# limanling/clip-event

Measured on AMD Instinct MI355X. Metric: image-text pairs/sec/GPU, ViT-B/32 224px x 77-tok, global-batch contrastive, higher is better.
Workload: dtype bf16; 1 GPU; ViT-B/32 224px x 77-tok, bf16 operands, per-GPU batch 256, K=1, InfoNCE only, full train step (fwd+bwd+clip_grad_norm+Adam), random-init weights; global_batch=256, parallelism=dp1, captions=SOT + U[8,75] random ids + EOT, zero-padded to 77 (SURVEY 8(d) c2), text_rows=live tokens SOT..EOT only: 54.8% of B*77 rows (identical results, see DESIGN.md), fresh_captions_every_step=True, alignment=False, cu_hog=0, nt_pgrid=256, full=False

## Files before the change

### clip_event_amd/csrc/attention.hip

```cpp
#include <map>
#include <mutex>

#include <type_traits>

#include "common.hpp"
#include "../../include/clip_event_hip.h"

namespace {

constexpr int HD = 64;
constexpr int ROW = 160;

typedef __attribute__((address_space(3))) s16x4 lds_s16x4;
typedef __attribute__((ext_vector_type(8))) short s16x8;

__device__ __forceinline__ bf16x8 tr_pair(const char* p0, const char* p1) {
    s16x4 lo = __builtin_amdgcn_ds_read_tr16_b64_v4i16((lds_s16x4*)p0);
    s16x4 hi = __builtin_amdgcn_ds_read_tr16_b64_v4i16((lds_s16x4*)p1);
    s16x8 v = {lo[0], lo[1], lo[2], lo[3], hi[0], hi[1], hi[2], hi[3]};
    return __builtin_bit_cast(bf16x8, v);
}

__device__ __forceinline__ bf16x8 pack8(const f32x4& a, const f32x4& b) {
    u32x4 v = {pack_bf2(a[0], a[1]), pack_bf2(a[2], a[3]), pack_bf2(b[0], b[1]), pack_bf2(b[2], b[3])};
    return __builtin_bit_cast(bf16x8, v);
}

template <int NCH>
__device__ __forceinline__ void stage_kv(char* sK, char* sV, const bf16_t* srcK, const bf16_t* srcV, long ld, int L, int Lp, int tid,
                                         int nthr) {
    const uint32_t span = (uint32_t)(((long)L - 1) * ld * 2 + HD * 2);
    const __amdgpu_buffer_rsrc_t rK = make_rsrc(srcK, span), rV = make_rsrc(srcV, span);
    u32x4 kv[NCH], vv[NCH];
#pragma unroll
    for (int j = 0; j < NCH; ++j) {
        const int idx = tid + j * nthr, r = idx >> 3, c = idx & 7;
        const uint32_t off = r < L ? (uint32_t)(r * ld * 2 + c * 16) : 0x80000000u;
        kv[j] = __builtin_amdgcn_raw_buffer_load_b128(rK, off, 0, 0);
        vv[j] = __builtin_amdgcn_raw_buffer_load_b128(rV, off, 0, 0);
    }
#pragma unroll
    for (int j = 0; j < NCH; ++j) {
        const int idx = tid + j * nthr, r = idx >> 3, c = idx & 7;
        if (idx < Lp * 8) {
            *reinterpret_cast<u32x4*>(sK + r * ROW + c * 16) = kv[j];
            *reinterpret_cast<u32x4*>(sV + r * ROW + c * 16) = vv[j];
        }
    }
}

template <int T>
__global__ __launch_bounds__(512) void attn_fwd_kernel(const bf16_t* __restrict__ qkv, long ld, bf16_t* __restrict__ o,
                                                       long ldo, float* __restrict__ lse,
                                                       const int* __restrict__ cu, int Lmax, int H, int D,
                                                       int causal, float scale) {
    extern __shared__ __attribute__((aligned(16))) char smem[];
    constexpr int Lp = T * 16;
    char* sK = smem;
    char* sV = smem + Lp * ROW;
    const int tid = threadIdx.x, lane = tid & 63;
    const int wave = __builtin_amdgcn_readfirstlane(tid >> 6), nw = blockDim.x >> 6;
    const int b = blockIdx.x / H, h = blockIdx.x - b * H;
    const long row0 = cu ? (long)cu[b] : (long)b * Lmax;
    const int L = cu ? min(cu[b + 1] - cu[b], Lmax) : Lmax;
    if (L <= 0) return;
    const int Tl = ((L + 31) >> 5) << 1;
    const bf16_t* base = qkv + row0 * ld + h * HD;

    const int li = lane & 15, g = lane >> 4;
    const int nstrips = (L + 15) >> 4;
    const int strip = wave;
    const int i = strip * 16 + li;
    const int iq = min(i, L - 1);
    bf16x8 qf[2];
    if (strip < nstrips) {
#pragma unroll
        for (int ks = 0; ks < 2; ++ks)
            qf[ks] = *reinterpret_cast<const bf16x8*>(base + (long)iq * ld + ks * 32 + g * 8);
    }
    stage_kv<4>(sK, sV, base + D, base + 2 * D, ld, L, Tl * 16, tid, blockDim.x);
    __syncthreads();

    if (strip < nstrips) {
        f32x4 s[T];
#pragma unroll
        for (int t = 0; t < T; ++t) {
            s[t] = f32x4{0.f, 0.f, 0.f, 0.f};
            if (t < Tl) {
#pragma unroll
                for (int ks = 0; ks < 2; ++ks) {
                    bf16x8 kf = *reinterpret_cast<const bf16x8*>(sK + (t * 16 + li) * ROW + (ks * 4 + g) * 16);
                    s[t] = __builtin_amdgcn_mfma_f32_16x16x32_bf16(kf, qf[ks], s[t], 0, 0, 0);
                }
            }
        }
        float mx = -INFINITY;
#pragma unroll
        for (int t = 0; t < T; ++t)
#pragma unroll
            for (int r = 0; r < 4; ++r) {
                const int j = t * 16 + g * 4 + r;
                const bool ok = (j < L) && (!causal || j <= i);
                s[t][r] = ok ? s[t][r] * scale : -INFINITY;
                mx = fmaxf(mx, s[t][r]);
            }
        mx = fmaxf(mx, __shfl_xor(mx, 16, 64));
        mx = fmaxf(mx, __shfl_xor(mx, 32, 64));
        float sum = 0.f;
#pragma unroll
        for (int t = 0; t < T; ++t)
#pragma unroll
            for (int r = 0; r < 4; ++r) {
                s[t][r] = __expf(s[t][r] - mx);
                sum += s[t][r];
            }
        sum += __shfl_xor(sum, 16, 64);
        sum += __shfl_xor(sum, 32, 64);
        f32x4 acc[4];
#pragma unroll
        for (int ct = 0; ct < 4; ++ct) acc[ct] = f32x4{0.f, 0.f, 0.f, 0.f};
#pragma unroll
        for (int sidx = 0; sidx < T / 2; ++sidx) {
            if (2 * sidx >= Tl) continue;
            bf16x8 pf = pack8(s[2 * sidx], s[2 * sidx + 1]);
            const char* vrow = sV + (32 * sidx + 4 * g + (li >> 2)) * ROW + (4 * (li & 3)) * 2;
#pragma unroll
            for (int ct = 0; ct < 4; ++ct) {
                bf16x8 vf = tr_pair(vrow + ct * 32, vrow + ct * 32 + 16 * ROW);
                acc[ct] = __builtin_amdgcn_mfma_f32_16x16x32_bf16(vf, pf, acc[ct], 0, 0, 0);
            }
        }
        if (i < L) {
            const float inv = 1.0f / sum;
            bf16_t* orow = o + (row0 + i) * ldo + h * HD + 4 * g;
#pragma unroll
            for (int ct = 0; ct < 4; ++ct) {
                u32x2 pk = {pack_bf2(acc[ct][0] * inv, acc[ct][1] * inv), pack_bf2(acc[ct][2] * inv, acc[ct][3] * inv)};
                *reinterpret_cast<u32x2*>(orow + ct * 16) = pk;
            }
            if (g == 0) lse[((long)b * H + h) * Lmax + i] = mx + __logf(sum);
        }
    }
}

template <int T>
__global__ __launch_bounds__(512) void attn_bwd_kernel(const bf16_t* __restrict__ qkv, long ld,
                                                       const bf16_t* __restrict__ o, long ldo,
                                                       const bf16_t* __restrict__ dout, long lddo,
                                                       const float* __restrict__ lse, bf16_t* __restrict__ dqkv,
                                                       long lddq, float* __restrict__ bias_grad,
                                                       const int* __restrict__ cu, int Lmax, int H, int D,
                                                       int causal, float scale) {
    extern __shared__ __attribute__((aligned(16))) char smem[];
    constexpr int Lp = T * 16;
    constexpr int PROW = Lp * 2 + 32;
    char* sA = smem;
    char* sB = sA + Lp * ROW;
    char* sP = sB + Lp * ROW;
    char* sDS = sP + Lp * PROW;
    auto csum = [&](int i) __attribute__((always_inline)) -> float* { return reinterpret_cast<float*>(sP + (i >> 3) * PROW + Lp * 2 + (i & 7) * 4); };
    const int tid = threadIdx.x, lane = tid & 63;
    const int wave = __builtin_amdgcn_readfirstlane(tid >> 6), nw = blockDim.x >> 6;
    const int b = blockIdx.x / H, h = blockIdx.x - b * H;
    const long row0 = cu ? (long)cu[b] : (long)b * Lmax;
    const int L = cu ? min(cu[b + 1] - cu[b], Lmax) : Lmax;
    if (L <= 0) return;
    const int Tl = ((L + 31) >> 5) << 1;
    const int Ll = Tl * 16;
    const bf16_t* base = qkv + row0 * ld + h * HD;
    const bf16_t* dob = dout + row0 * lddo + h * HD;
    const bf16_t* ob = o + row0 * ldo + h * HD;
    bf16_t* dbase = dqkv + row0 * lddq + h * HD;

    for (int i = tid; i < 192; i += blockDim.x) *csum(i) = 0.f;
    const int li = lane & 15, g = lane >> 4;
    u32x4 rK[2], rV[2], rQ[2], rD[2];
#pragma unroll
    for (int c = 0; c < 2; ++c) {
        const int idx = tid + c * blockDim.x;
        const int r = idx >> 3, ch = idx & 7;
        const u32x4 z = {0u, 0u, 0u, 0u};
        rK[c] = z; rV[c] = z; rQ[c] = z; rD[c] = z;
        if (idx < Ll * 8 && r < L) {
            rK[c] = *reinterpret_cast<const u32x4*>(base + D + (long)r * ld + ch * 8);
            rV[c] = *reinterpret_cast<const u32x4*>(base + 2 * D + (long)r * ld + ch * 8);
            rQ[c] = *reinterpret_cast<const u32x4*>(base + (long)r * ld + ch * 8);
            rD[c] = *reinterpret_cast<const u32x4*>(dob + (long)r * lddo + ch * 8);
        }
    }
    const int strip = wave;
    const bool has_strip = strip < Tl;
    const int i = strip * 16 + li;
    const bool iok = has_strip && i < L;
    const int iq = min(i, L - 1);
    float dl = 0.f, lsei = 0.f;
    bf16x8 qf[2], df[2];
    if (has_strip) {
        const u32x4* pd = reinterpret_cast<const u32x4*>(dob + (long)iq * lddo + g * 16);
        const u32x4* po = reinterpret_cast<const u32x4*>(ob + (long)iq * ldo + g * 16);
#pragma unroll
        for (int v = 0; v < 2; ++v) {
            u32x4 a = pd[v], c = po[v];
#pragma unroll
            for (int e = 0; e < 4; ++e) dl += bf_lo(a[e]) * bf_lo(c[e]) + bf_hi(a[e]) * bf_hi(c[e]);
        }
        lsei = lse[((long)b * H + h) * Lmax + iq];
#pragma unroll
        for (int ks = 0; ks < 2; ++ks) {
            qf[ks] = *reinterpret_cast<const bf16x8*>(base + (long)iq * ld + ks * 32 + g * 8);
            df[ks] = *reinterpret_cast<const bf16x8*>(dob + (long)iq * lddo + ks * 32 + g * 8);
        }
    }
#pragma unroll
    for (int c = 0; c < 2; ++c) {
        const int idx = tid + c * blockDim.x;
        if (idx < Ll * 8) {
            *reinterpret_cast<u32x4*>(sA + (idx >> 3) * ROW + (idx & 7) * 16) = rK[c];
            *reinterpret_cast<u32x4*>(sB + (idx >> 3) * ROW + (idx & 7) * 16) = rV[c];
        }
    }
    __syncthreads();
    dl += __shfl_xor(dl, 16, 64);
    dl += __shfl_xor(dl, 32, 64);

    if (has_strip) {
        f32x4 p[T], ds[T];
#pragma unroll
        for (int t = 0; t < T; ++t) {
            p[t] = f32x4{0.f, 0.f, 0.f, 0.f};
            ds[t] = f32x4{0.f, 0.f, 0.f, 0.f};
            if (t >= Tl) continue;
#pragma unroll
            for (int ks = 0; ks < 2; ++ks) {
                bf16x8 kf = *reinterpret_cast<const bf16x8*>(sA + (t * 16 + li) * ROW + (ks * 4 + g) * 16);
                bf16x8 vf = *reinterpret_cast<const bf16x8*>(sB + (t * 16 + li) * ROW + (ks * 4 + g) * 16);
                p[t] = __builtin_amdgcn_mfma_f32_16x16x32_bf16(kf, qf[ks], p[t], 0, 0, 0);
                ds[t] = __builtin_amdgcn_mfma_f32_16x16x32_bf16(vf, df[ks], ds[t], 0, 0, 0);
            }
#pragma unroll
            for (int r = 0; r < 4; ++r) {
                const int j = t * 16 + g * 4 + r;
                const bool ok = iok && (j < L) && (!causal || j <= i);
                const float pv = ok ? __expf(p[t][r] * scale - lsei) : 0.f;
                p[t][r] = pv;
                ds[t][r] = pv * (ds[t][r] - dl) * scale;
            }
            u32x2 pk = {pack_bf2(p[t][0], p[t][1]), pack_bf2(p[t][2], p[t][3])};
            u32x2 dk = {pack_bf2(ds[t][0], ds[t][1]), pack_bf2(ds[t][2], ds[t][3])};
            *reinterpret_cast<u32x2*>(sP + i * PROW + (t * 16 + g * 4) * 2) = pk;
            *reinterpret_cast<u32x2*>(sDS + i * PROW + (t * 16 + g * 4) * 2) = dk;
        }
        f32x4 acc[4];
#pragma unroll
        for (int ct = 0; ct < 4; ++ct) acc[ct] = f32x4{0.f, 0.f, 0.f, 0.f};
#pragma unroll
        for (int sidx = 0; sidx < T / 2; ++sidx) {
            if (2 * sidx >= Tl) continue;
            bf16x8 sf = pack8(ds[2 * sidx], ds[2 * sidx + 1]);
            const char* krow = sA + (32 * sidx + 4 * g + (li >> 2)) * ROW + (4 * (li & 3)) * 2;
#pragma unroll
            for (int ct = 0; ct < 4; ++ct) {
                bf16x8 kf = tr_pair(krow + ct * 32, krow + ct * 32 + 16 * ROW);
                acc[ct] = __builtin_amdgcn_mfma_f32_16x16x32_bf16(kf, sf, acc[ct], 0, 0, 0);
            }
        }
        if (iok) {
            bf16_t* qrow = dbase + (long)i * lddq + 4 * g;
#pragma unroll
            for (int ct = 0; ct < 4; ++ct) {
                u32x2 pk = {pack_bf2(acc[ct][0], acc[ct][1]), pack_bf2(acc[ct][2], acc[ct][3])};
                *reinterpret_cast<u32x2*>(qrow + ct * 16) = pk;
            }
        }
        if (bias_grad) {
            float vals[16];
#pragma unroll
            for (int ct = 0; ct < 4; ++ct)
#pragma unroll
                for (int r = 0; r < 4; ++r) vals[ct * 4 + r] = acc[ct][r];
            const float tot = row16_colsum(vals, li);
            const int k = row16_colsum_index(li);
            atomicAdd(csum((k >> 2) * 16 + 4 * g + (k & 3)), tot);
        }
    }
    __syncthreads();
#pragma unroll
    for (int c = 0; c < 2; ++c) {
        const int idx = tid + c * blockDim.x;
        if (idx < Ll * 8) {
            *reinterpret_cast<u32x4*>(sA + (idx >> 3) * ROW + (idx & 7) * 16) = rQ[c];
            *reinterpret_cast<u32x4*>(sB + (idx >> 3) * ROW + (idx & 7) * 16) = rD[c];
        }
    }
    __syncthreads();
    const int nkt = (L + 15) >> 4;
    for (int jt = wave; jt < nkt; jt += nw) {
        const int j = jt * 16 + li;
        f32x4 av[4], ak[4];
#pragma unroll
        for (int ct = 0; ct < 4; ++ct) {
            av[ct] = f32x4{0.f, 0.f, 0.f, 0.f};
            ak[ct] = f32x4{0.f, 0.f, 0.f, 0.f};
        }
#pragma unroll
        for (int sidx = 0; sidx < T / 2; ++sidx) {
            if (2 * sidx >= Tl) continue;
            const int irow = 32 * sidx + 8 * g + (li >> 2);
            const char* pcol = sP + irow * PROW + (jt * 16 + 4 * (li & 3)) * 2;
            const char* scol = sDS + irow * PROW + (jt * 16 + 4 * (li & 3)) * 2;
            bf16x8 pf = tr_pair(pcol, pcol + 4 * PROW);
            bf16x8 sf = tr_pair(scol, scol + 4 * PROW);
            const int roff = irow * ROW + (4 * (li & 3)) * 2;
#pragma unroll
            for (int ct = 0; ct < 4; ++ct) {
                bf16x8 dof = tr_pair(sB + roff + ct * 32, sB + roff + ct * 32 + 4 * ROW);
                bf16x8 qf = tr_pair(sA + roff + ct * 32, sA + roff + ct * 32 + 4 * ROW);
                av[ct] = __builtin_amdgcn_mfma_f32_16x16x32_bf16(dof, pf, av[ct], 0, 0, 0);
                ak[ct] = __builtin_amdgcn_mfma_f32_16x16x32_bf16(qf, sf, ak[ct], 0, 0, 0);
            }
        }
        if (j < L) {
            bf16_t* krow = dbase + (long)j * lddq + D + 4 * g;
            bf16_t* vrow = dbase + (long)j * lddq + 2 * D + 4 * g;
#pragma unroll
            for (int ct = 0; ct < 4; ++ct) {
                u32x2 pk = {pack_bf2(ak[ct][0], ak[ct][1]), pack_bf2(ak[ct][2], ak[ct][3])};
                u32x2 pv = {pack_bf2(av[ct][0], av[ct][1]), pack_bf2(av[ct][2], av[ct][3])};
                *reinterpret_cast<u32x2*>(krow + ct * 16) = pk;
                *reinterpret_cast<u32x2*>(vrow + ct * 16) = pv;
            }
        }
        if (bias_grad) {
            float vk[16], vv[16];
#pragma unroll
            for (int ct = 0; ct < 4; ++ct)
#pragma unroll
                for (int r = 0; r < 4; ++r) {
                    vk[ct * 4 + r] = ak[ct][r];
                    vv[ct * 4 + r] = av[ct][r];
                }
            const float tk = row16_colsum(vk, li), tv = row16_colsum(vv, li);
            const int k = row16_colsum_index(li);
            atomicAdd(csum(64 + (k >> 2) * 16 + 4 * g + (k & 3)), tk);
            atomicAdd(csum(128 + (k >> 2) * 16 + 4 * g + (k & 3)), tv);
        }
    }
    if (bias_grad) {
        __syncthreads();
        for (int i = tid; i < 192; i += blockDim.x) atomicAdd(bias_grad + (i >> 6) * D + h * HD + (i & 63), *csum(i));
    }
}

constexpr int LB = 64;
constexpr int LPROW = LB * 2 + 32;

__device__ __forceinline__ void stage_block(char* dst, const bf16_t* src, long ld, int row0, int L, int tid) {
#pragma unroll
    for (int c = 0; c < 2; ++c) {
        const int idx = tid + c * 256;
        const int r = idx >> 3, ch = idx & 7;
        u32x4 v = {0u, 0u, 0u, 0u};
        if (row0 + r < L) v = *reinterpret_cast<const u32x4*>(src + (long)(row0 + r) * ld + ch * 8);
        *reinterpret_cast<u32x4*>(dst + r * ROW + ch * 16) = v;
    }
}

struct BlockRegs { u32x4 v[2]; };
__device__ __forceinline__ BlockRegs load_block(const bf16_t* src, long ld, int row0, int L, int tid) {
    BlockRegs b;
#pragma unroll
    for (int c = 0; c < 2; ++c) {
        const int idx = tid + c * 256;
        const int r = idx >> 3, ch = idx & 7;
        b.v[c] = u32x4{0u, 0u, 0u, 0u};
        if (row0 + r < L) b.v[c] = *reinterpret_cast<const u32x4*>(src + (long)(row0 + r) * ld + ch * 8);
    }
    return b;
}
__device__ __forceinline__ void store_block(char* dst, const BlockRegs& b, int tid) {
#pragma unroll
    for (int c = 0; c < 2; ++c) {
        const int idx = tid + c * 256;
        *reinterpret_cast<u32x4*>(dst + (idx >> 3) * ROW + (idx & 7) * 16) = b.v[c];
    }
}

__device__ __forceinline__ void long_block_coords(int xcd_order, int& blk, int& bh) {
    blk = blockIdx.x;
    bh = blockIdx.y;
    const int nblk = gridDim.x, nbh = gridDim.y;
    if (xcd_order && (nbh & 7) == 0) {
        const int id = blockIdx.y * nblk + blockIdx.x;
        const int xcd = id & 7, slot = id >> 3;
        bh = (slot / nblk) * 8 + xcd;
        blk = slot - (slot / nblk) * nblk;
    }
}

template <int NS>
__global__ __launch_bounds__(256) void attn_fwd_long_kernel(const bf16_t* __restrict__ qkv, long ld, bf16_t* __restrict__ o,
                                                            long ldo, float* __restrict__ lse, int L, int H, int D,
                                                            int causal, float scale, int xcd_order) {
    __shared__ __attribute__((aligned(16))) char smem[2 * LB * ROW];
    char* sK = smem;
    char* sV = smem + LB * ROW;
    const int tid = threadIdx.x, lane = tid & 63;
    const int wave = __builtin_amdgcn_readfirstlane(tid >> 6);
    int qb, bh_;
    long_block_coords(xcd_order, qb, bh_);
    const int b = bh_ / H, h = bh_ - b * H;
    const bf16_t* base = qkv + (long)b * L * ld + h * HD;
    const int li = lane & 15, g = lane >> 4;
    constexpr int QB = LB * NS;
    int i[NS];
    bf16x8 qf[NS][2];
    float m[NS], l[NS];
    f32x4 acc[NS][4];
#pragma unroll
    for (int s = 0; s < NS; ++s) {
        i[s] = qb * QB + (wave * NS + s) * 16 + li;
        const int iq = min(i[s], L - 1);
#pragma unroll
        for (int ks = 0; ks < 2; ++ks) qf[s][ks] = *reinterpret_cast<const bf16x8*>(base + (long)iq * ld + ks * 32 + g * 8);
        m[s] = -INFINITY;
        l[s] = 0.f;
#pragma unroll
        for (int ct = 0; ct < 4; ++ct) acc[s][ct] = f32x4{0.f, 0.f, 0.f, 0.f};
    }
    const float c2 = scale * 1.4426950408889634f;
    const int nkb_all = (L + LB - 1) / LB;
    const int nkb = causal ? min(nkb_all, (qb * QB + QB - 1) / LB + 1) : nkb_all;
    BlockRegs nk = load_block(base + D, ld, 0, L, tid), nv = load_block(base + 2 * D, ld, 0, L, tid);
    for (int kb = 0; kb < nkb; ++kb) {
        if (kb) __syncthreads();
        store_block(sK, nk, tid);
        store_block(sV, nv, tid);
        if (kb + 1 < nkb) {
            nk = load_block(base + D, ld, (kb + 1) * LB, L, tid);
            nv = load_block(base + 2 * D, ld, (kb + 1) * LB, L, tid);
        }
        __syncthreads();
        f32x4 sc[NS][4];
        const bool need_mask = causal || (kb + 1) * LB > L;
#pragma unroll
        for (int t = 0; t < 4; ++t) {
// ... 533 lines not shown
```

### clip_event_amd/csrc/layernorm.hip

```cpp
#include <stdlib.h>

#include "common.hpp"
#include "../../include/clip_event_hip.h"

namespace {

__device__ __forceinline__ __amdgpu_buffer_rsrc_t row_rsrc(const void* base, long row, long ld, int esz, int D) {
    return make_rsrc(reinterpret_cast<const char*>(base) + row * ld * esz, (uint32_t)(D * esz));
}
#ifndef CE_LN_NT
#define CE_LN_NT 0
#endif
template <int T> struct Raw4 { typedef u32x2 type; };
template <> struct Raw4<CE_T_F32> { typedef f32x4 type; };
template <int T, int AUX = 0>
__device__ __forceinline__ typename Raw4<T>::type ld4_row(__amdgpu_buffer_rsrc_t r, int c) {
    if constexpr (T == CE_T_F32) return __builtin_bit_cast(f32x4, __builtin_amdgcn_raw_buffer_load_b128(r, c * 4, 0, AUX));
    else return __builtin_amdgcn_raw_buffer_load_b64(r, c * 2, 0, AUX);
}
template <int T>
__device__ __forceinline__ f32x4 cvt4(typename Raw4<T>::type raw) {
    if constexpr (T == CE_T_F32) return raw;
    else if constexpr (T == CE_T_F16) return f16x4_to_f32(raw);
    else return f32x4{bf_lo(raw[0]), bf_hi(raw[0]), bf_lo(raw[1]), bf_hi(raw[1])};
// ... 121 lines not shown
    for (int i = 0; i < IT; ++i) {
        aw[i] = f32x4{0.f, 0.f, 0.f, 0.f};
        ab[i] = f32x4{0.f, 0.f, 0.f, 0.f};
        ax[i] = f32x4{0.f, 0.f, 0.f, 0.f};
    }
    const float invD = 1.0f / (float)D;
    const float gscale = gscale_ptr ? *gscale_ptr : 1.0f;
    const float dy_mul = DYT == CE_T_F16 ? 1.0f / gscale : 1.0f;
    const float din_mul = DIT == CE_T_F16 ? 1.0f / gscale : 1.0f;
    const float out_mul = DOT == CE_T_F16 ? gscale : 1.0f;
    float om = 0.f;
#ifndef CE_LN_PFD
#define CE_LN_PFD 1
#endif
    constexpr int PFD = !PF ? 1 : ((NW >= 16 && XT == CE_T_F32 && DYT == CE_T_F32) ? 1 : CE_LN_PFD);
    struct Pending {
        typename Raw4<XT>::type xr[IT];
        typename Raw4<DYT>::type dr[IT];
        typename Raw4<DIT>::type ir[IT];
        float mu, rs;
        int dst;
    };
    Pending pend[PFD];
    f32x4 gw[IT];
    {
        const __amdgpu_buffer_rsrc_t rw = make_rsrc(w, (uint32_t)(D * 4));
#pragma unroll
        for (int i = 0; i < IT; ++i) gw[i] = ld4_row<CE_T_F32>(rw, i * 256 + lane * 4);
    }
    constexpr int XB = XT == CE_T_F32 ? 4 : 2, DYB = DYT == CE_T_F32 ? 4 : 2, DIB = DIT == CE_T_F32 ? 4 : 2, DOB = DOT == CE_T_F32 ? 4 : 2;
    auto fetch = [&](Pending& P, int r) __attribute__((always_inline)) {
        P.dst = __builtin_amdgcn_readfirstlane(rows ? rows[r] : r);
        P.mu = mean[r];
        P.rs = rstd[r];
        const __amdgpu_buffer_rsrc_t rx = row_rsrc(x, P.dst, ldx, XB, D), rdy = row_rsrc(dy, r, lddy, DYB, D);
#pragma unroll
        for (int i = 0; i < IT; ++i) {
            P.xr[i] = ld4_row<XT, CE_LN_NT>(rx, i * 256 + lane * 4);
            P.dr[i] = ld4_row<DYT, CE_LN_NT>(rdy, i * 256 + lane * 4);
        }
        if (dx_in) {
            const __amdgpu_buffer_rsrc_t rin = row_rsrc(dx_in, P.dst, lddx, DIB, D);
#pragma unroll
            for (int i = 0; i < IT; ++i) P.ir[i] = ld4_row<DIT, CE_LN_NT>(rin, i * 256 + lane * 4);
        }
    };
    const int stride = gridDim.x * NW;
    auto consume = [&](Pending& P, int next) __attribute__((always_inline)) {
        const int cdst = P.dst;
        const float cmu = P.mu, crs = P.rs;
        f32x4 xh[IT], gy[IT], din[IT];
        float s1 = 0.f, s2 = 0.f;
#pragma unroll
        for (int i = 0; i < IT; ++i) {
            const f32x4 xv = cvt4<XT>(P.xr[i]);
            f32x4 d = cvt4<DYT>(P.dr[i]);
            if constexpr (DYT == CE_T_F16) d *= dy_mul;
            din[i] = f32x4{0.f, 0.f, 0.f, 0.f};
            if (dx_in) {
                din[i] = cvt4<DIT>(P.ir[i]);
                if constexpr (DIT == CE_T_F16) din[i] *= din_mul;
            }
            xh[i] = (xv - cmu) * crs;
            gy[i] = d * gw[i];
            aw[i] += d * xh[i];
            ab[i] += d;
            s1 += (gy[i][0] + gy[i][1]) + (gy[i][2] + gy[i][3]);
            f32x4 t = gy[i] * xh[i];
            s2 += (t[0] + t[1]) + (t[2] + t[3]);
        }
        if constexpr (PF) {
            if (next < M) fetch(P, next);
        }
        const float c1 = wave_sum_dpp(s1) * invD, c2 = wave_sum_dpp(s2) * invD;
        u32x2 pkq[IT];
        const __amdgpu_buffer_rsrc_t ro = row_rsrc(dx_out, cdst, lddx, DOB, D);
        const __amdgpu_buffer_rsrc_t rb = row_rsrc(dxb ? (const void*)dxb : (const void*)dx_out, cdst, lddxb, 2, dxb ? D : 0);
#pragma unroll
        for (int i = 0; i < IT; ++i) {
            const int c = i * 256 + lane * 4;
            f32x4 o = (gy[i] - c1 - xh[i] * c2) * crs + din[i];
            o = (c < D) ? o : f32x4{0.f, 0.f, 0.f, 0.f};
            ax[i] += o;
            if constexpr (DOT == CE_T_F16) {
                const f32x4 os = o * out_mul;
                om = absmax4(om, os);
                st4_row<DOT, CE_LN_NT>(ro, c, os);
            } else {
                st4_row<DOT, CE_LN_NT>(ro, c, o);
            }
            pkq[i] = u32x2{pack_bf2(o[0], o[1]), pack_bf2(o[2], o[3])};
            __builtin_amdgcn_raw_buffer_store_b64(pkq[i], rb, c * 2, 0, CE_LN_NT);
        }
        if (q8) quant_row_from_regs<IT>(pkq, lane, D, q8 + (long)cdst * ldq, qscale + cdst);
        if constexpr (!PF) {
            if (next < M) fetch(P, next);
        }
    };
    const int r0 = blockIdx.x * NW + wave;
#pragma unroll
    for (int k = 0; k < PFD; ++k)
        if (r0 + k * stride < M) fetch(pend[k], r0 + k * stride);
    for (int r = r0; r < M; r += PFD * stride) {
#pragma unroll
        for (int k = 0; k < PFD; ++k)
            if (r + k * stride < M) consume(pend[k], r + (k + PFD) * stride);
    }
    if constexpr (DOT == CE_T_F16) {
        if (sat && !(om < CE_F16_LIMIT)) atomicAdd(sat + 1, 1u);
    }
    const int P = dxsum ? 3 : 2;
    float* strip = red + NW * D;
#pragma unroll
    for (int pass = 0; pass < 3; ++pass) {
        if (pass >= P) break;
        __syncthreads();
#pragma unroll
        for (int i = 0; i < IT; ++i) {
            const int c = i * 256 + lane * 4;
            if (c < D) *reinterpret_cast<f32x4*>(&red[wave * D + c]) = pass == 0 ? aw[i] : (pass == 1 ? ab[i] : ax[i]);
        }
        __syncthreads();
        for (int c = threadIdx.x; c < D; c += 64 * NW) {
            float t = 0.f;
#pragma unroll
            for (int wv = 0; wv < NW; ++wv) t += red[wv * D + c];
            strip[pass * D + c] = t;
        }
    }
    __syncthreads();
    const int total = P * D;
    if (partial) {
        float* pp = partial + (size_t)blockIdx.x * 3 * D;
        for (int j = threadIdx.x; j < total; j += 64 * NW) pp[j] = strip[j];
        return;
    }
    const int start = (int)((blockIdx.x * 64u) % (unsigned)total);
    for (int j = threadIdx.x; j < total; j += 64 * NW) {
        int e = j + start;
        if (e >= total) e -= total;
        const int pass = e >= 2 * D ? 2 : (e >= D ? 1 : 0);
        float* dstp = pass == 0 ? dw : (pass == 1 ? db : dxsum);
#ifndef CE_DIAG_LN_NO_ATOMICS
        atomicAdd(dstp + (e - pass * D), strip[e]);
#else
        if (strip[e] == 123.456f) dstp[e - pass * D] = strip[e];
#endif
    }
}

struct LnFoldJobs {
    ce_ln_fold_job job[CE_LN_FOLD_MAX];
};
__global__ __launch_bounds__(256) void ln_fold_kernel(LnFoldJobs jobs) {
    const ce_ln_fold_job& jb = jobs.job[blockIdx.y];
    const int D = jb.D, P = jb.dxsum ? 3 : 2;
    const int j = blockIdx.x * 256 + threadIdx.x;
    if (j >= P * D) return;
    float t = 0.f;
    const float* pp = jb.partials + j;
#pragma unroll 8
    for (int b = 0; b < jb.blocks; ++b) t += pp[(size_t)b * 3 * D];
    const int pass = j / D, c = j - pass * D;
    float* dst = pass == 0 ? jb.dw : (pass == 1 ? jb.db : jb.dxsum);
    dst[c] += t;
}

}

#define LN_DISPATCH(D, CALL)                                     \
    do {                                                         \
        if ((D) <= 256) { CALL(1); }                             \
        else if ((D) <= 512) { CALL(2); }                        \
        else if ((D) <= 768) { CALL(3); }                        \
        else if ((D) <= 1024) { CALL(4); }                       \
        else { CALL(8); }                                        \
    } while (0)

extern "C" int ce_layernorm_fwd_t(const void* x, int x_type, long ldx, const int* rows, const float* w, const float* b,
                                  void* y, int y_type, long ldy, float* mean, float* rstd, int M, int D, float eps,
                                  void* stream) {
    return ce_layernorm_fwd_q8(x, x_type, ldx, rows, w, b, y, y_type, ldy, mean, rstd, M, D, eps, nullptr, 0, nullptr, stream);
}

extern "C" int ce_layernorm_fwd_q8(const void* x, int x_type, long ldx, const int* rows, const float* w, const float* b,
                                   void* y, int y_type, long ldy, float* mean, float* rstd, int M, int D, float eps,
                                   void* q8v, long ldq, float* qscale, void* stream) {
    uint8_t* q8 = reinterpret_cast<uint8_t*>(q8v);
    CE_CHECK_ARG(!q8 || (y_type == CE_T_BF16 && qscale && ldq >= D && ldq % 4 == 0), "ce_layernorm_fwd_q8: the e4m3 copy needs a bf16 output, scales and ldq >= D");
    CE_CHECK_ARG(M > 0 && D > 0 && D % 4 == 0 && D <= 2048, "ce_layernorm_fwd: need 0<D<=2048, D%%4==0 (D=%d M=%d)", D, M);
    CE_CHECK_ARG(ldx % 4 == 0 && ldy % 4 == 0, "ce_layernorm_fwd: leading dimensions must be multiples of 4");
    static const int rpw_env = getenv("CE_LN_FWD_RPW") ? atoi(getenv("CE_LN_FWD_RPW")) : 0;
    const int rpw = D > 1024 ? 1 : (rpw_env == 2 ? 2 : 1);
    dim3 grid(ce_div_up(M, 4 * rpw)), block(256);
    hipStream_t s = (hipStream_t)stream;
    unsigned int* sat = ce_sat_counters();
    CeProfScope prof(CE_PROF_LN_FWD, 8.0 * M * D, (double)(ce_type_bytes(x_type) + ce_type_bytes(y_type)) * M * D, s);
    const int combo = x_type * 4 + y_type;
#define CALL(IT)                                                                                                              \
    switch (combo) {                                                                                                          \
        case CE_T_F32 * 4 + CE_T_BF16: if (rpw == 2 && IT <= 4) hipLaunchKernelGGL((ln_fwd_kernel<IT, CE_T_F32, CE_T_BF16, (IT <= 4 ? 2 : 1)>), grid, block, 0, s, x, ldx, rows, w, b, y, ldy, mean, rstd, M, D, eps, q8, ldq, qscale, sat); else hipLaunchKernelGGL((ln_fwd_kernel<IT, CE_T_F32, CE_T_BF16, 1>), grid, block, 0, s, x, ldx, rows, w, b, y, ldy, mean, rstd, M, D, eps, q8, ldq, qscale, sat); break; \
        case CE_T_F32 * 4 + CE_T_F32: if (rpw == 2 && IT <= 4) hipLaunchKernelGGL((ln_fwd_kernel<IT, CE_T_F32, CE_T_F32, (IT <= 4 ? 2 : 1)>), grid, block, 0, s, x, ldx, rows, w, b, y, ldy, mean, rstd, M, D, eps, q8, ldq, qscale, sat); else hipLaunchKernelGGL((ln_fwd_kernel<IT, CE_T_F32, CE_T_F32, 1>), grid, block, 0, s, x, ldx, rows, w, b, y, ldy, mean, rstd, M, D, eps, q8, ldq, qscale, sat); break;   \
        case CE_T_F32 * 4 + CE_T_F16: if (rpw == 2 && IT <= 4) hipLaunchKernelGGL((ln_fwd_kernel<IT, CE_T_F32, CE_T_F16, (IT <= 4 ? 2 : 1)>), grid, block, 0, s, x, ldx, rows, w, b, y, ldy, mean, rstd, M, D, eps, q8, ldq, qscale, sat); else hipLaunchKernelGGL((ln_fwd_kernel<IT, CE_T_F32, CE_T_F16, 1>), grid, block, 0, s, x, ldx, rows, w, b, y, ldy, mean, rstd, M, D, eps, q8, ldq, qscale, sat); break;   \
        case CE_T_F16 * 4 + CE_T_BF16: if (rpw == 2 && IT <= 4) hipLaunchKernelGGL((ln_fwd_kernel<IT, CE_T_F16, CE_T_BF16, (IT <= 4 ? 2 : 1)>), grid, block, 0, s, x, ldx, rows, w, b, y, ldy, mean, rstd, M, D, eps, q8, ldq, qscale, sat); else hipLaunchKernelGGL((ln_fwd_kernel<IT, CE_T_F16, CE_T_BF16, 1>), grid, block, 0, s, x, ldx, rows, w, b, y, ldy, mean, rstd, M, D, eps, q8, ldq, qscale, sat); break; \
        case CE_T_F16 * 4 + CE_T_F32: if (rpw == 2 && IT <= 4) hipLaunchKernelGGL((ln_fwd_kernel<IT, CE_T_F16, CE_T_F32, (IT <= 4 ? 2 : 1)>), grid, block, 0, s, x, ldx, rows, w, b, y, ldy, mean, rstd, M, D, eps, q8, ldq, qscale, sat); else hipLaunchKernelGGL((ln_fwd_kernel<IT, CE_T_F16, CE_T_F32, 1>), grid, block, 0, s, x, ldx, rows, w, b, y, ldy, mean, rstd, M, D, eps, q8, ldq, qscale, sat); break;   \
        case CE_T_F16 * 4 + CE_T_F16: if (rpw == 2 && IT <= 4) hipLaunchKernelGGL((ln_fwd_kernel<IT, CE_T_F16, CE_T_F16, (IT <= 4 ? 2 : 1)>), grid, block, 0, s, x, ldx, rows, w, b, y, ldy, mean, rstd, M, D, eps, q8, ldq, qscale, sat); else hipLaunchKernelGGL((ln_fwd_kernel<IT, CE_T_F16, CE_T_F16, 1>), grid, block, 0, s, x, ldx, rows, w, b, y, ldy, mean, rstd, M, D, eps, q8, ldq, qscale, sat); break;   \
        default: CE_CHECK_ARG(false, "ce_layernorm_fwd: element types x=%d y=%d are not built (x: f32 / f16, y: bf16 / f32 / f16)", x_type, y_type); \
    }
    LN_DISPATCH(D, CALL);
#undef CALL
    CE_LAUNCH_CHECK();
    return 0;
}

extern "C" int ce_layernorm_fwd(const float* x, long ldx, const int* rows, const float* w, const float* b, void* y,
                                long ldy, int out_f32, float* mean, float* rstd, int M, int D, float eps,
                                void* stream) {
    return ce_layernorm_fwd_t(x, CE_T_F32, ldx, rows, w, b, y, out_f32 ? CE_T_F32 : CE_T_BF16, ldy, mean, rstd, M, D, eps,
                              stream);
}

extern "C" int ce_layernorm_bwd_t(const void* dy, int dy_type, long lddy, const void* x, int x_type, long ldx,
                                  const int* rows, const float* mean, const float* rstd, const float* w,
                                  const void* dx_in, int dxin_type, void* dx_out, int dx_type, long lddx, void* dxb,
                                  long lddxb, float* dw, float* db, float* dxsum, const float* gscale, int M, int D,
                                  void* stream) {
    return ce_layernorm_bwd_q8(dy, dy_type, lddy, x, x_type, ldx, rows, mean, rstd, w, dx_in, dxin_type, dx_out, dx_type, lddx, dxb,
                               lddxb, dw, db, dxsum, gscale, M, D, nullptr, 0, nullptr, stream);
}

static int ln_bwd_blocks(int M, int D) {
    const int nw = D <= 512 ? 16 : (D <= 1024 ? 8 : 4);
    int blocks = ce_div_up(M, nw);
    static const int cap = getenv("CE_LN_BWD_BLOCKS") ? atoi(getenv("CE_LN_BWD_BLOCKS")) : 256;
    return blocks > cap ? cap : blocks;
}
extern "C" int ce_layernorm_bwd_blocks(int M, int D) { return ln_bwd_blocks(M, D); }

static int ln_bwd_launch(const void* dy, int dy_type, long lddy, const void* x, int x_type, long ldx,
                         const int* rows, const float* mean, const float* rstd, const float* w,
                         const void* dx_in, int dxin_type, void* dx_out, int dx_type, long lddx, void* dxb,
                         long lddxb, float* dw, float* db, float* dxsum, const float* gscale, int M, int D,
                         void* q8v, long ldq, float* qscale, float* partial, void* stream);

extern "C" int ce_layernorm_bwd_q8(const void* dy, int dy_type, long lddy, const void* x, int x_type, long ldx,
                                   const int* rows, const float* mean, const float* rstd, const float* w,
                                   const void* dx_in, int dxin_type, void* dx_out, int dx_type, long lddx, void* dxb,
                                   long lddxb, float* dw, float* db, float* dxsum, const float* gscale, int M, int D,
                                   void* q8v, long ldq, float* qscale, void* stream) {
    return ln_bwd_launch(dy, dy_type, lddy, x, x_type, ldx, rows, mean, rstd, w, dx_in, dxin_type, dx_out, dx_type, lddx, dxb, lddxb, dw, db,
                         dxsum, gscale, M, D, q8v, ldq, qscale, nullptr, stream);
}

extern "C" int ce_layernorm_bwd_partials(const void* dy, int dy_type, long lddy, const void* x, int x_type, long ldx,
                                         const int* rows, const float* mean, const float* rstd, const float* w,
                                         const void* dx_in, int dxin_type, void* dx_out, int dx_type, long lddx, void* dxb,
                                         long lddxb, int want_dxsum, const float* gscale, int M, int D, void* q8v, long ldq,
                                         float* qscale, float* partials, void* stream) {
    CE_CHECK_ARG(partials, "ce_layernorm_bwd_partials: null partials buffer");
    float* tag = partials;
    return ln_bwd_launch(dy, dy_type, lddy, x, x_type, ldx, rows, mean, rstd, w, dx_in, dxin_type, dx_out, dx_type, lddx, dxb, lddxb, tag, tag,
                         want_dxsum ? tag : nullptr, gscale, M, D, q8v, ldq, qscale, partials, stream);
}

extern "C" int ce_layernorm_fold(const ce_ln_fold_job* jobs, int njobs, void* stream) {
    CE_CHECK_ARG(jobs && njobs > 0, "ce_layernorm_fold: no jobs");
    for (int base = 0; base < njobs; base += CE_LN_FOLD_MAX) {
        LnFoldJobs pack;
        const int n = njobs - base < CE_LN_FOLD_MAX ? njobs - base : CE_LN_FOLD_MAX;
        int maxd = 0;
        for (int i = 0; i < n; ++i) {
            pack.job[i] = jobs[base + i];
            CE_CHECK_ARG(pack.job[i].partials && pack.job[i].dw && pack.job[i].db && pack.job[i].blocks > 0 && pack.job[i].D > 0,
                         "ce_layernorm_fold: job %d incomplete", base + i);
            if (pack.job[i].D > maxd) maxd = pack.job[i].D;
        }
        hipLaunchKernelGGL(ln_fold_kernel, dim3(ce_div_up(3 * maxd, 256), n), dim3(256), 0, (hipStream_t)stream, pack);
    }
    CE_LAUNCH_CHECK();
    return 0;
}

static int ln_bwd_launch(const void* dy, int dy_type, long lddy, const void* x, int x_type, long ldx,
                         const int* rows, const float* mean, const float* rstd, const float* w,
                         const void* dx_in, int dxin_type, void* dx_out, int dx_type, long lddx, void* dxb,
                         long lddxb, float* dw, float* db, float* dxsum, const float* gscale, int M, int D,
                         void* q8v, long ldq, float* qscale, float* partial, void* stream) {
    uint8_t* q8 = reinterpret_cast<uint8_t*>(q8v);
    CE_CHECK_ARG(!q8 || (dxb && qscale && ldq >= D && ldq % 4 == 0), "ce_layernorm_bwd_q8: the e4m3 copy is a copy of dxb (needs dxb, scales, ldq >= D)");
    CE_CHECK_ARG(M > 0 && D > 0 && D % 4 == 0 && D <= 2048, "ce_layernorm_bwd: need 0<D<=2048, D%%4==0 (D=%d M=%d)", D, M);
    CE_CHECK_ARG(lddy % 4 == 0 && ldx % 4 == 0 && lddx % 4 == 0 && lddxb % 4 == 0, "ce_layernorm_bwd: leading dimensions must be multiples of 4");
    if (!dx_in) dxin_type = CE_T_F32;
    CE_CHECK_ARG(gscale || (dy_type != CE_T_F16 && dxin_type != CE_T_F16 && dx_type != CE_T_F16),
                 "ce_layernorm_bwd: an fp16 gradient operand needs the device scale (ce_grad_scale)");
    const int nw = D <= 512 ? 16 : (D <= 1024 ? 8 : 4);
    const int blocks = ln_bwd_blocks(M, D);
    dim3 grid(blocks), block(64 * nw);
    const size_t lds = (size_t)(nw + 3) * D * sizeof(float);
    hipStream_t s = (hipStream_t)stream;
    unsigned int* sat = ce_sat_counters();
    CeProfScope prof(CE_PROF_LN_BWD, 16.0 * M * D,
                     (double)(ce_type_bytes(dy_type) + ce_type_bytes(x_type) + (dx_in ? ce_type_bytes(dxin_type) : 0) +
                              ce_type_bytes(dx_type) + (dxb ? 2 : 0)) * M * D, s);
    const int combo = ((dy_type * 4 + x_type) * 4 + dxin_type) * 4 + dx_type;
#define LNB(DYT, XT, DIT, DOT) (((DYT * 4 + XT) * 4 + DIT) * 4 + DOT)
#define LAUNCH(IT, DYT, XT, DIT, DOT)                                                                                         \
    hipLaunchKernelGGL((ln_bwd_kernel<IT, (IT <= 2 ? 16 : (IT <= 4 ? 8 : 4)), DYT, XT, DIT, DOT, true>), grid, block, lds, s, dy, lddy, \
                       x, ldx, rows, mean, rstd, w, dx_in, dx_out, lddx, (bf16_t*)dxb, lddxb, dw, db, dxsum, gscale, M, D, q8, ldq, qscale, partial, sat)
#define CALL(IT)                                                                                                              \
    switch (combo) {                                                                                                          \
        case LNB(CE_T_BF16, CE_T_F32, CE_T_F32, CE_T_F32): LAUNCH(IT, CE_T_BF16, CE_T_F32, CE_T_F32, CE_T_F32); break;        \
        case LNB(CE_T_F32, CE_T_F32, CE_T_F32, CE_T_F32): LAUNCH(IT, CE_T_F32, CE_T_F32, CE_T_F32, CE_T_F32); break;          \
        case LNB(CE_T_BF16, CE_T_F16, CE_T_F16, CE_T_F16): LAUNCH(IT, CE_T_BF16, CE_T_F16, CE_T_F16, CE_T_F16); break;        \
        case LNB(CE_T_BF16, CE_T_F16, CE_T_F32, CE_T_F16): LAUNCH(IT, CE_T_BF16, CE_T_F16, CE_T_F32, CE_T_F16); break;        \
        case LNB(CE_T_BF16, CE_T_F16, CE_T_F32, CE_T_F32): LAUNCH(IT, CE_T_BF16, CE_T_F16, CE_T_F32, CE_T_F32); break;        \
        case LNB(CE_T_BF16, CE_T_F16, CE_T_F16, CE_T_F32): LAUNCH(IT, CE_T_BF16, CE_T_F16, CE_T_F16, CE_T_F32); break;        \
        case LNB(CE_T_F16, CE_T_F32, CE_T_F32, CE_T_F32): LAUNCH(IT, CE_T_F16, CE_T_F32, CE_T_F32, CE_T_F32); break;          \
        case LNB(CE_T_F16, CE_T_F16, CE_T_F32, CE_T_F32): LAUNCH(IT, CE_T_F16, CE_T_F16, CE_T_F32, CE_T_F32); break;          \
        default: CE_CHECK_ARG(false, "ce_layernorm_bwd: element types dy=%d x=%d dx_in=%d dx_out=%d are not built", dy_type, \
                              x_type, dxin_type, dx_type);                                                                    \
    }
    LN_DISPATCH(D, CALL);
#undef CALL
#undef LAUNCH
#undef LNB
    CE_LAUNCH_CHECK();
    return 0;
}

extern "C" int ce_layernorm_bwd(const void* dy, long lddy, int dy_f32, const float* x, long ldx, const int* rows,
                                const float* mean, const float* rstd, const float* w, const float* dx_in,
                                float* dx_out, long lddx, void* dxb, long lddxb, float* dw, float* db, float* dxsum, int M,
                                int D, void* stream) {
    return ce_layernorm_bwd_t(dy, dy_f32 ? CE_T_F32 : CE_T_BF16, lddy, x, CE_T_F32, ldx, rows, mean, rstd, w, dx_in, CE_T_F32,
                              dx_out, CE_T_F32, lddx, dxb, lddxb, dw, db, dxsum, nullptr, M, D, stream);
}
```

Baseline: 20940 pairs/s (whole job).

## Use buffer loads with early-issued prefetch in attention bwd and split LN fold reduction

The attention backward kernel now loads K/V, Q/dO fragments, LSE and O through raw buffer loads with out-of-range offsets in place of branches. All global loads are issued up front, with Q/dO staging deferred behind a vmcnt wait, so their latency overlaps the first MFMA phase. The layernorm fold kernel is restructured so each block handles 32 columns with 32 slices of partial rows in parallel, batched 8 deep, then reduced through LDS. This replaces the long serial per-thread loop. The cost is more register pressure from holding prefetched data and a hand-coded waitcnt constant that depends on the target.

```diff
diff --git a/clip_event_amd/csrc/attention.hip b/clip_event_amd/csrc/attention.hip
--- a/clip_event_amd/csrc/attention.hip
+++ b/clip_event_amd/csrc/attention.hip
@@ -10,6 +10,7 @@
 
 constexpr int HD = 64;
 constexpr int ROW = 160;
+constexpr int WAIT_VMCNT0 = 0x0F70;
 
 typedef __attribute__((address_space(3))) s16x4 lds_s16x4;
 typedef __attribute__((ext_vector_type(8))) short s16x8;
@@ -166,7 +167,6 @@
     const int L = cu ? min(cu[b + 1] - cu[b], Lmax) : Lmax;
     if (L <= 0) return;
     const int Tl = ((L + 31) >> 5) << 1;
-    const int Ll = Tl * 16;
     const bf16_t* base = qkv + row0 * ld + h * HD;
     const bf16_t* dob = dout + row0 * lddo + h * HD;
     const bf16_t* ob = o + row0 * ldo + h * HD;
@@ -174,55 +174,75 @@
 
     for (int i = tid; i < 192; i += blockDim.x) *csum(i) = 0.f;
     const int li = lane & 15, g = lane >> 4;
-    u32x4 rK[2], rV[2], rQ[2], rD[2];
-#pragma unroll
-    for (int c = 0; c < 2; ++c) {
-        const int idx = tid + c * blockDim.x;
-        const int r = idx >> 3, ch = idx & 7;
-        const u32x4 z = {0u, 0u, 0u, 0u};
-        rK[c] = z; rV[c] = z; rQ[c] = z; rD[c] = z;
-        if (idx < Ll * 8 && r < L) {
-            rK[c] = *reinterpret_cast<const u32x4*>(base + D + (long)r * ld + ch * 8);
-            rV[c] = *reinterpret_cast<const u32x4*>(base + 2 * D + (long)r * ld + ch * 8);
-            rQ[c] = *reinterpret_cast<const u32x4*>(base + (long)r * ld + ch * 8);
-            rD[c] = *reinterpret_cast<const u32x4*>(dob + (long)r * lddo + ch * 8);
-        }
-    }
+    constexpr uint32_t OOR = 0x80000000u;
+    const uint32_t span_q = (uint32_t)(((long)L - 1) * ld * 2 + HD * 2), span_d = (uint32_t)(((long)L - 1) * lddo * 2 + HD * 2);
+    const __amdgpu_buffer_rsrc_t dsQ = make_rsrc(base, span_q), dsK = make_rsrc(base + D, span_q), dsV = make_rsrc(base + 2 * D, span_q);
+    const __amdgpu_buffer_rsrc_t dsD = make_rsrc(dob, span_d), dsO = make_rsrc(ob, (uint32_t)(((long)L - 1) * ldo * 2 + HD * 2));
+    const __amdgpu_buffer_rsrc_t dsL = make_rsrc(lse + ((long)b * H + h) * Lmax, (uint32_t)L * 4u);
     const int strip = wave;
     const bool has_strip = strip < Tl;
     const int i = strip * 16 + li;
     const bool iok = has_strip && i < L;
     const int iq = min(i, L - 1);
-    float dl = 0.f, lsei = 0.f;
-    bf16x8 qf[2], df[2];
-    if (has_strip) {
-        const u32x4* pd = reinterpret_cast<const u32x4*>(dob + (long)iq * lddo + g * 16);
-        const u32x4* po = reinterpret_cast<const u32x4*>(ob + (long)iq * ldo + g * 16);
-#pragma unroll
-        for (int v = 0; v < 2; ++v) {
-            u32x4 a = pd[v], c = po[v];
-#pragma unroll
-            for (int e = 0; e < 4; ++e) dl += bf_lo(a[e]) * bf_lo(c[e]) + bf_hi(a[e]) * bf_hi(c[e]);
-        }
-        lsei = lse[((long)b * H + h) * Lmax + iq];
-#pragma unroll
-        for (int ks = 0; ks < 2; ++ks) {
-            qf[ks] = *reinterpret_cast<const bf16x8*>(base + (long)iq * ld + ks * 32 + g * 8);
-            df[ks] = *reinterpret_cast<const bf16x8*>(dob + (long)iq * lddo + ks * 32 + g * 8);
-        }
-    }
+    uint32_t tq[2], td[2];
 #pragma unroll
     for (int c = 0; c < 2; ++c) {
         const int idx = tid + c * blockDim.x;
-        if (idx < Ll * 8) {
-            *reinterpret_cast<u32x4*>(sA + (idx >> 3) * ROW + (idx & 7) * 16) = rK[c];
-            *reinterpret_cast<u32x4*>(sB + (idx >> 3) * ROW + (idx & 7) * 16) = rV[c];
-        }
+        const int r = idx >> 3, ch = idx & 7;
+        tq[c] = r < L ? (uint32_t)(r * ld * 2 + ch * 16) : OOR;
+        td[c] = r < L ? (uint32_t)(r * lddo * 2 + ch * 16) : OOR;
+    }
+    const uint32_t fq = has_strip ? (uint32_t)(iq * ld * 2 + g * 16) : OOR;
+    const uint32_t fd = has_strip ? (uint32_t)(iq * lddo * 2 + g * 16) : OOR;
+    const uint32_t fo = has_strip ? (uint32_t)(iq * ldo * 2 + g * 32) : OOR;
+    u32x4 rK[2], rV[2], rQ[2], rD[2];
+#pragma unroll
+    for (int c = 0; c < 2; ++c) {
+        rK[c] = __builtin_amdgcn_raw_buffer_load_b128(dsK, tq[c], 0, 0);
+        rV[c] = __builtin_amdgcn_raw_buffer_load_b128(dsV, tq[c], 0, 0);
+    }
+    __builtin_amdgcn_sched_barrier(0);
+    bf16x8 qf[2], df[2];
+#pragma unroll
+    for (int ks = 0; ks < 2; ++ks) {
+        qf[ks] = __builtin_bit_cast(bf16x8, __builtin_amdgcn_raw_buffer_load_b128(dsQ, fq + ks * 64, 0, 0));
+        df[ks] = __builtin_bit_cast(bf16x8, __builtin_amdgcn_raw_buffer_load_b128(dsD, fd + ks * 64, 0, 0));
+    }
+    const float lsei = __uint_as_float(__builtin_amdgcn_raw_buffer_load_b32(dsL, has_strip ? (uint32_t)iq * 4u : OOR, 0, 0));
+    u32x4 da[2], oa[2];
+#pragma unroll
+    for (int v = 0; v < 2; ++v) {
+        da[v] = __builtin_amdgcn_raw_buffer_load_b128(dsD, fd + g * 16 + v * 16, 0, 0);
+        oa[v] = __builtin_amdgcn_raw_buffer_load_b128(dsO, fo + v * 16, 0, 0);
+    }
+    __builtin_amdgcn_sched_barrier(0);
+#pragma unroll
+    for (int c = 0; c < 2; ++c) {
+        rQ[c] = __builtin_amdgcn_raw_buffer_load_b128(dsQ, tq[c], 0, 0);
+        rD[c] = __builtin_amdgcn_raw_buffer_load_b128(dsD, td[c], 0, 0);
+    }
+    __builtin_amdgcn_sched_barrier(0);
+#pragma unroll
+    for (int c = 0; c < 2; ++c) {
+        const int idx = tid + c * blockDim.x;
+        *reinterpret_cast<u32x4*>(sA + (idx >> 3) * ROW + (idx & 7) * 16) = rK[c];
+        *reinterpret_cast<u32x4*>(sB + (idx >> 3) * ROW + (idx & 7) * 16) = rV[c];
     }
     __syncthreads();
+    __builtin_amdgcn_sched_barrier(0);
+    float dl = 0.f;
+#pragma unroll
+    for (int v = 0; v < 2; ++v) {
+        const u32x4 a = da[v], c = oa[v];
+#pragma unroll
+        for (int e = 0; e < 4; ++e) dl += bf_lo(a[e]) * bf_lo(c[e]) + bf_hi(a[e]) * bf_hi(c[e]);
+    }
     dl += __shfl_xor(dl, 16, 64);
     dl += __shfl_xor(dl, 32, 64);
 
+    f32x4 acc[4];
+#pragma unroll
+    for (int ct = 0; ct < 4; ++ct) acc[ct] = f32x4{0.f, 0.f, 0.f, 0.f};
     if (has_strip) {
         f32x4 p[T], ds[T];
 #pragma unroll
@@ -250,9 +270,6 @@
             *reinterpret_cast<u32x2*>(sP + i * PROW + (t * 16 + g * 4) * 2) = pk;
             *reinterpret_cast<u32x2*>(sDS + i * PROW + (t * 16 + g * 4) * 2) = dk;
         }
-        f32x4 acc[4];
-#pragma unroll
-        for (int ct = 0; ct < 4; ++ct) acc[ct] = f32x4{0.f, 0.f, 0.f, 0.f};
 #pragma unroll
         for (int sidx = 0; sidx < T / 2; ++sidx) {
             if (2 * sidx >= Tl) continue;
@@ -264,6 +281,10 @@
                 acc[ct] = __builtin_amdgcn_mfma_f32_16x16x32_bf16(kf, sf, acc[ct], 0, 0, 0);
             }
         }
+    }
+    __builtin_amdgcn_wave_barrier();
+    __builtin_amdgcn_s_waitcnt(WAIT_VMCNT0);
+    if (has_strip) {
         if (iok) {
             bf16_t* qrow = dbase + (long)i * lddq + 4 * g;
 #pragma unroll
@@ -287,10 +308,8 @@
 #pragma unroll
     for (int c = 0; c < 2; ++c) {
         const int idx = tid + c * blockDim.x;
-        if (idx < Ll * 8) {
-            *reinterpret_cast<u32x4*>(sA + (idx >> 3) * ROW + (idx & 7) * 16) = rQ[c];
-            *reinterpret_cast<u32x4*>(sB + (idx >> 3) * ROW + (idx & 7) * 16) = rD[c];
-        }
+        *reinterpret_cast<u32x4*>(sA + (idx >> 3) * ROW + (idx & 7) * 16) = rQ[c];
+        *reinterpret_cast<u32x4*>(sB + (idx >> 3) * ROW + (idx & 7) * 16) = rD[c];
     }
     __syncthreads();
     const int nkt = (L + 15) >> 4;
diff --git a/clip_event_amd/csrc/layernorm.hip b/clip_event_amd/csrc/layernorm.hip
--- a/clip_event_amd/csrc/layernorm.hip
+++ b/clip_event_amd/csrc/layernorm.hip
@@ -297,18 +297,38 @@
 struct LnFoldJobs {
     ce_ln_fold_job job[CE_LN_FOLD_MAX];
 };
-__global__ __launch_bounds__(256) void ln_fold_kernel(LnFoldJobs jobs) {
+constexpr int FOLD_COLS = 32, FOLD_SLICES = 32, FOLD_BATCH = 8;
+__global__ __launch_bounds__(FOLD_COLS * FOLD_SLICES) void ln_fold_kernel(LnFoldJobs jobs) {
+    __shared__ float part[FOLD_SLICES][FOLD_COLS];
     const ce_ln_fold_job& jb = jobs.job[blockIdx.y];
-    const int D = jb.D, P = jb.dxsum ? 3 : 2;
-    const int j = blockIdx.x * 256 + threadIdx.x;
-    if (j >= P * D) return;
+    const int D = jb.D, P = jb.dxsum ? 3 : 2, blocks = jb.blocks;
+    if ((int)blockIdx.x * FOLD_COLS >= P * D) return;
+    const int col = threadIdx.x & (FOLD_COLS - 1), slice = threadIdx.x / FOLD_COLS;
+    const int j = blockIdx.x * FOLD_COLS + col;
+    const bool live = j < P * D;
     float t = 0.f;
-    const float* pp = jb.partials + j;
-#pragma unroll 8
-    for (int b = 0; b < jb.blocks; ++b) t += pp[(size_t)b * 3 * D];
-    const int pass = j / D, c = j - pass * D;
-    float* dst = pass == 0 ? jb.dw : (pass == 1 ? jb.db : jb.dxsum);
-    dst[c] += t;
+    for (int b0 = 0; b0 < blocks; b0 += FOLD_SLICES * FOLD_BATCH) {
+        const int rows = min(blocks - b0, FOLD_SLICES * FOLD_BATCH);
+        const __amdgpu_buffer_rsrc_t rp = make_rsrc(jb.partials + (size_t)b0 * 3 * D, (uint32_t)rows * 3u * (uint32_t)D * 4u);
+        float v[FOLD_BATCH];
+#pragma unroll
+        for (int k = 0; k < FOLD_BATCH; ++k) {
+            const int b = slice + k * FOLD_SLICES;
+            v[k] = __uint_as_float(__builtin_amdgcn_raw_buffer_load_b32(rp, live && b < rows ? ((uint32_t)b * 3u * D + j) * 4u : 0x80000000u, 0, 0));
+        }
+#pragma unroll
+        for (int k = 0; k < FOLD_BATCH; ++k) t += v[k];
+    }
+    part[slice][col] = t;
+    __syncthreads();
+    if (threadIdx.x < FOLD_COLS && live) {
+        float tot = 0.f;
+#pragma unroll
+        for (int s = 0; s < FOLD_SLICES; ++s) tot += part[s][col];
+        const int pass = j / D, c = j - pass * D;
+        float* dst = pass == 0 ? jb.dw : (pass == 1 ? jb.db : jb.dxsum);
+        dst[c] += tot;
+    }
 }
 
 }
@@ -420,7 +440,7 @@
                          "ce_layernorm_fold: job %d incomplete", base + i);
             if (pack.job[i].D > maxd) maxd = pack.job[i].D;
         }
-        hipLaunchKernelGGL(ln_fold_kernel, dim3(ce_div_up(3 * maxd, 256), n), dim3(256), 0, (hipStream_t)stream, pack);
+        hipLaunchKernelGGL(ln_fold_kernel, dim3(ce_div_up(3 * maxd, FOLD_COLS), n), dim3(FOLD_COLS * FOLD_SLICES), 0, (hipStream_t)stream, pack);
     }
     CE_LAUNCH_CHECK();
     return 0;
```

Measured after the change: 21080 pairs/s (whole job) (median of 6 runs). About the same (+0.7%).
